# nipponjo/tts-arabic-pytorch

Hardware: AMD Instinct MI355X
Metric: audio samples/sec (FastPitch+HiFi-GAN, synthetic 64-phoneme inputs) (higher is better)
Workload: dtype f32

## Files before the change

### include/ttsamd.h

```cpp
#ifndef TTSAMD_H
#define TTSAMD_H

#include <stdint.h>

#ifdef __cplusplus
extern "C" {
#endif

#define TTSAMD_OK 0
#define TTSAMD_EINVAL (-1)
#define TTSAMD_EHIP (-2)
#define TTSAMD_ENOMEM (-3)

typedef struct ttsamd_tensor {
    const char* name;
    const float* data;
    int32_t ndim;
    int64_t shape[4];
} ttsamd_tensor;

typedef struct ttsamd_hifigan_cfg {
    int32_t num_mels;
    int32_t upsample_initial_channel;
    int32_t n_ups;
// ... 260 lines not shown

int64_t ttsamd_conv1d_packed_floats(int32_t cout, int32_t cin, int32_t k);
int32_t ttsamd_conv1d(const float* x, const float* w, const float* bias, const int64_t* lens,
                      int32_t batch, int32_t cin, int32_t cout, int32_t k, int32_t dilation,
                      int32_t lin, float in_slope, int32_t relu_out, float* y, float* packed,
                      void* stream);
int32_t ttsamd_conv1d_ex(const float* x, const float* w, const float* bias, const float* res, const int64_t* lens, int32_t batch,
                         int32_t cin, int32_t cout, int32_t k, int32_t dilation, int32_t lin, float in_slope,
                         int32_t relu_out, int32_t mode, float div, float* y, float* packed, void* stream);
int32_t ttsamd_conv1d_splitk(const float* x, const float* w, const float* bias, const float* res, const int64_t* lens, int32_t batch,
                             int32_t cin, int32_t cout, int32_t k, int32_t dilation, int32_t lin, float in_slope,
                             int32_t relu_out, int32_t mode, float div, float* y, float* packed, float* splitk_ws, int64_t splitk_floats,
                             void* stream);
int32_t ttsamd_conv_last_launch(int32_t* route, int32_t* ksplit);
int64_t ttsamd_convt_packed_floats(int32_t cin, int32_t cout, int32_t u);
int32_t ttsamd_conv_transpose1d(const float* x, const float* w, const float* bias, const int64_t* lens, int32_t batch, int32_t cin,
                                int32_t cout, int32_t u, int32_t lin, float in_slope, float* y, float* packed, void* stream);

int64_t ttsamd_resblock_pair_packed_floats(int32_t channels, int32_t k, int32_t variant);
int32_t ttsamd_resblock_pair(const float* x, float* y, const float* w1, const float* b1, const float* w2, const float* b2,
                             int32_t channels, int32_t k, int32_t dil, const int64_t* lens, int32_t len_mul, int32_t L,
                             int32_t batch, int32_t mode, float div, float slope, int32_t variant, float* packed, int64_t packed_floats,
                             void* stream);

int64_t ttsamd_resblock2_packed_floats(int32_t channels, int32_t k, int32_t variant);
int32_t ttsamd_resblock2(const float* x, float* y, const float* w1, const float* b1, const float* w2, const float* b2, int32_t channels,
                         int32_t k, int32_t dil1, int32_t dil2, const int64_t* lens, int32_t len_mul, int32_t L, int32_t batch, int32_t mode,
                         float div, float slope, int32_t variant, float* packed, int64_t packed_floats, void* stream);

int32_t ttsamd_bfo_pack(const float* x, int32_t batch, int32_t channels, int32_t len, float slope, void* out, void* stream);
// ... 97 lines not shown
```

### tts-arabic-pytorch_amd/csrc/api.hip

```cpp
#include <cerrno>
#include <cstdio>
#include <cstdlib>
#include <cstring>
#include <algorithm>
#include <atomic>
#include <mutex>
#include <string>
#include <vector>

#include "kernels.hpp"

namespace ttsamd {

static thread_local std::string g_err;

void set_error(const char* fmt, ...) {
    char buf[1024];
    va_list ap;
    va_start(ap, fmt);
    vsnprintf(buf, sizeof(buf), fmt, ap);
    va_end(ap);
    g_err = buf;
}

// ... 158 lines not shown

__global__ void pack_convt_weight_kernel(const float* __restrict__ w, int cin, int cout, int u, int cp, float* __restrict__ out) {
    const int64_t i = (int64_t)blockIdx.x * 256 + threadIdx.x;
    const int64_t n = (int64_t)u * cin * 2 * cp;
    if (i >= n) return;
    const int pq = (int)(i % 4);
    const int co = (int)((i / 4) % cp);
    const int kk = (int)((i / (4 * (int64_t)cp)) % 2);
    const int t = (int)((i / (8 * (int64_t)cp)) % 2);
    const int o = (int)((i / (16 * (int64_t)cp)) % (cin / 8));
    const int rho = (int)(i / (16 * (int64_t)cp * (cin / 8)));
    const int kidx = (rho + u / 2) % u + t * u;
    out[i] = co < cout ? w[((int64_t)(8 * o + 2 * pq + kk) * cout + co) * (2 * u) + kidx] : 0.f;
}

__global__ void split_bf16_kernel(const float* __restrict__ packed, int64_t n, unsigned short* __restrict__ out) {
    const int64_t i = (int64_t)blockIdx.x * 256 + threadIdx.x;
    if (i >= n) return;
    const float f = packed[i];
    unsigned u = __float_as_uint(f);
    u += 0x7fffu + ((u >> 16) & 1u);
    const unsigned h = u >> 16;
    const float r = f - __uint_as_float(h << 16);
    unsigned v = __float_as_uint(r);
    v += 0x7fffu + ((v >> 16) & 1u);
    out[i] = (unsigned short)h;
    out[n + i] = (unsigned short)(v >> 16);
}

namespace {
// ... 645 lines not shown

int32_t ttsamd_conv1d(const float* x, const float* w, const float* bias, const int64_t* lens, int32_t batch,
                      int32_t cin, int32_t cout, int32_t k, int32_t dilation, int32_t lin, float in_slope,
                      int32_t relu_out, float* y, float* packed, void* stream) {
    return ttsamd_conv1d_ex(x, w, bias, nullptr, lens, batch, cin, cout, k, dilation, lin, in_slope, relu_out, 0, 1.f, y, packed, stream);
}

int32_t ttsamd_conv_last_launch(int32_t* route, int32_t* ksplit) {
    TTS_REQUIRE(route && ksplit, "conv_last_launch: null argument");
    last_conv_launch(route, ksplit);
    return 0;
}

int64_t ttsamd_convt_packed_floats(int32_t cin, int32_t cout, int32_t u) {
    if (cin < 1 || cout < 1 || u < 1) return 0;
    return 2 * (int64_t)u * cin * 2 * cout_padded(cout);
}

int32_t ttsamd_conv_transpose1d(const float* x, const float* w, const float* bias, const int64_t* lens, int32_t batch, int32_t cin,
                                int32_t cout, int32_t u, int32_t lin, float in_slope, float* y, float* packed, void* stream) {
    TTS_REQUIRE(x && w && y && packed, "conv_transpose1d: null argument");
    TTS_REQUIRE(batch >= 1 && cin >= 8 && cin % 8 == 0 && cout >= 1 && lin >= 1, "conv_transpose1d: batch %d, cin %d (a multiple of 8), cout %d, lin %d",
                batch, cin, cout, lin);
    TTS_REQUIRE(u >= 2 && u % 2 == 0, "conv_transpose1d: stride %d (kernel 2 u, padding u / 2: u even)", u);
    TTS_REQUIRE((int64_t)lin * u < ((int64_t)1 << 31) / 4 / cout, "conv_transpose1d: %d x %d x %d outputs per row", cout, lin, u);
    hipStream_t s = (hipStream_t)stream;
    const int cp = cout_padded(cout);
    const int64_t n = (int64_t)u * cin * 2 * cp;
    hipLaunchKernelGGL(pack_convt_weight_kernel, dim3((unsigned)((n + 255) / 256)), dim3(256), 0, s, w, cin, cout, u, cp, packed);
    TTS_CHECK_HIP(hipGetLastError());
    unsigned short* planes = nullptr;
    if (default_precision() != 0) {
        planes = reinterpret_cast<unsigned short*>(packed + n);
        hipLaunchKernelGGL(split_bf16_kernel, dim3((unsigned)((n + 255) / 256)), dim3(256), 0, s, packed, n, planes);
        TTS_CHECK_HIP(hipGetLastError());
    }
    ConvParams p;
    std::memset(&p, 0, sizeof(p));
    p.batch = batch;
    p.lens_in = lens; p.lens_out = lens;
    prof_begin(s, 2.0 * cout * cin * 2 * u);
    const int32_t rc = launch_upsampler(p, x, packed, planes, bias, y, cin, cout, u, 2 * u, lin, 1, in_slope, opt_int(OPT_CONVT, 1) != 0, s);
    prof_end(s);
    return rc;
}

int64_t ttsamd_resblock_pair_packed_floats(int32_t channels, int32_t k, int32_t variant) {
    if (channels < 1 || k < 1) return 0;
    const int64_t n = 2 * (int64_t)channels * k * channels;
    const int nwino = (variant == 4 ? 1 : (variant == 5 ? 2 : 0));
    if (variant == 6) return n + ((k == 3 || k == 7 || k == 11) ? 2 * (int64_t)channels * wino4_groups(k) * channels : 0);
    return n + ((k == 3 || k == 7 || k == 11) ? nwino * (int64_t)channels * wino2_groups(k) * channels : 0);
}

int32_t ttsamd_resblock_pair(const float* x, float* y, const float* w1, const float* b1, const float* w2, const float* b2,
                             int32_t channels, int32_t k, int32_t dil, const int64_t* lens, int32_t len_mul, int32_t L,
                             int32_t batch, int32_t mode, float div, float slope, int32_t variant, float* packed, int64_t packed_floats,
// ... 151 lines not shown
```

### tts-arabic-pytorch_amd/csrc/common.hpp

```cpp
#pragma once
#include <hip/hip_runtime.h>
#include <stdint.h>
#include <atomic>
#include <cstdarg>
#include <cstdio>
#include <cstdlib>
#include <string>

#include "../../include/ttsamd.h"

namespace ttsamd {

void set_error(const char* fmt, ...);

#define TTS_CHECK_HIP(expr)                                                         \
    do {                                                                            \
        hipError_t e_ = (expr);                                                     \
        if (e_ != hipSuccess) {                                                     \
            ttsamd::set_error("%s failed: %s (%s:%d)", #expr, hipGetErrorString(e_), \
                              __FILE__, __LINE__);                                  \
            return TTSAMD_EHIP;                                                     \
        }                                                                           \
    } while (0)

// ... 23 lines not shown
    return e;
}

#define TTS_OPTIONS(X)                                                                                     \
    X(HIFIGAN_STREAMS, 0, 0, 1)    \
    X(WINO, 0, 0, 1)                                              \
    X(WINO2, 0, 0, 31)             \
    X(WINO4, 0, 0, 127)            \
    X(FUSED_PAIR, 0, 0, 1)                   \
    X(FUSED2, 0, 0, 1)                                           \
    X(FUSED2_MASK, 1, 0, 0x1ff)               \
    X(FUSED2_MASK_N1, 1, 0, 0x1ff)          \
    X(FUSED2_WB, 0, 0, 2)                     \
    X(PAIR4, 0, 0, 1)              \
    X(CONVT, 0, 0, 1)                              \
    X(BFO, 0, 0, 1)                \
    X(BFO_CHAIN, 0, 0, 1)                           \
    X(BFO_CHAIN7, 0, 0, 1)                                 \
    X(BFO_FF, 0, 0, 1)                              \
    X(BFO_SPLITK, 0, 0, 1)                                              \
    X(BFO_SMALL_TILES, 0, 0, 1)            \
    X(BF16_ATTN, 0, 0, 1)                                         \
    X(BF16_PACKED_T, 0, 0, 1)                   \
    X(ATT_RA, 0, 1, 4)                             \
    X(ATT_SPLIT, 0, 0, 1)                      \
    X(XCD_W, 0, 0, 1)                            \
    X(XCD_WMAX_KB, 0, 0, 1 << 20)     \
    X(DEEP_SPLITK, 0, 0, 1)        \
    X(TACO_PERSISTENT, 0, 0, 2)    \
    X(TACO_SEG, 0, 8, 1 << 20)     \
// ... 64 lines not shown
    unsigned long long* timing;
    const float* w_wino44;
};
constexpr int64_t kSplitKFloats = 4 << 20;
constexpr int64_t kSplitKFloatsFp = 8 << 20;

void conv_log(const char* kind, int K, int cin, int cout, int nout, int batch, int has_res, int mode, int len_mul, int ragged,
              int n_phase);
bool compact_order(const void* lens, int batch);
int32_t launch_conv(const ConvParams& p, hipStream_t stream);
void note_conv_launch(int32_t route, int32_t ksplit);
void last_conv_launch(int32_t* route, int32_t* ksplit);
bool convt_supported(const ConvParams& p);
int32_t launch_convt(const ConvParams& p, hipStream_t stream);
int32_t launch_upsampler(ConvParams& p, const float* x, const float* w, const void* w_bf16, const float* bias, float* y, int cin, int cout,
                         int u, int kt, int L, int len_mul, float in_slope, bool convt_ok, hipStream_t stream);
bool fused_pair_supported(int32_t channels, int32_t k, int32_t dil, int32_t L, const float* x, const float* y);
int32_t launch_fused_pair(int32_t channels, const float* x, float* y, const float* w1, const float* b1, const float* w2,
                          const float* b2, int32_t k, int32_t dil, const int64_t* lens, int32_t len_mul, int32_t L, int32_t batch,
                          int32_t mode, float div, float slope, hipStream_t stream);
bool fused_pair2_supported(int32_t channels, int32_t k, int32_t dil, int32_t L, const float* x, const float* y, int32_t ntw);
int32_t launch_fused_pair2(int32_t channels, const float* x, float* y, const float* w1, const float* b1, const float* w2,
                           const float* b2, int32_t k, int32_t dil, const int64_t* lens, int32_t len_mul, int32_t L, int32_t batch,
                           int32_t mode, float div, float slope, int32_t ntw, hipStream_t stream, const float* w2_wino = nullptr,
                           const float* w1_wino = nullptr);
bool fused_pair4_supported(int32_t channels, int32_t k, int32_t dil, int32_t L, const float* x, const float* y);
int32_t launch_fused_pair4(int32_t channels, const float* x, float* y, const float* w1_wino4, const float* b1, const float* w2_wino4,
                           const float* b2, int32_t k, int32_t dil, const int64_t* lens, int32_t len_mul, int32_t L, int32_t batch,
                           int32_t mode, float div, float slope, hipStream_t stream);
bool resblock2_conv_supported(int32_t channels, int32_t k, int32_t dil, int32_t L, const float* x, const float* y);
int32_t launch_resblock2_conv(int32_t channels, const float* x, float* y, const float* w, const float* b, int32_t k, int32_t dil,
// ... 17 lines not shown
int wino4_block_outputs(int dil);
int wino4_ksplit(const ConvParams& p);
int32_t launch_splitk_reduce(const ConvParams& q, hipStream_t stream);
int32_t launch_wino4(const ConvParams& p, hipStream_t stream);
void wino4_filter_groups(const float* g, int k, float* o);
void pack_wino4_weight(const float* w, int cout, int cin, int k, float* out);
void wino44_filter_groups(const float* g, int k, float* o);
void pack_wino44_weight(const float* w, int cout, int cin, int k, float* out);
void pack_conv_weight(const float* w, int cout, int cin, int k, float* out);
void pack_convt_weight(const float* w, int cin, int cout, int kt, int u, int p, float* out);
inline int cout_padded(int cout) { return (int)align_up(cout, 32); }
void split_packed_bf16(const float* packed, int64_t n, uint16_t* out);
int32_t default_precision();

#ifdef __HIPCC__
__device__ __forceinline__ bool live_tile(const int64_t* __restrict__ lens, const int mul, const int n_max, const int tile_w,
                                          const int batch, const unsigned lin, int& b, int& tile) {
    const int lane = threadIdx.x & 63;
    unsigned base = 0;
    for (int u0 = 0; u0 < batch; u0 += 64) {
        int n = 0;
        if (u0 + lane < batch) n = (max(min(n_max, (int)lens[u0 + lane] * mul), 0) + tile_w - 1) / tile_w;
        int incl = n;
#pragma unroll
        for (int d = 1; d < 64; d <<= 1) {
            const int t = __shfl_up(incl, d, 64);
            if (lane >= d) incl += t;
        }
        const unsigned total = (unsigned)__shfl(incl, 63, 64);
        if (lin < base + total) {
            const unsigned long long m = __ballot(base + (unsigned)incl > lin);
            const int l = __ffsll((long long)m) - 1;
            b = u0 + l;
            tile = (int)(lin - base) - (__shfl(incl, l, 64) - __shfl(n, l, 64));
            return true;
        }
        base += total;
// ... 7 lines not shown
```

### tts-arabic-pytorch_amd/csrc/conv_wino4.hip

```cpp
#include <cstdlib>
#include <cstring>

#include <algorithm>
#include <vector>

#include "conv_mfma_common.hpp"
#include "bfo.hpp"

namespace ttsamd {

typedef float w4_f32x4 __attribute__((ext_vector_type(4)));
typedef float w4_f32x2 __attribute__((ext_vector_type(2)));

template <int K, int NOCT_, int NSTAGE_, int PT_ = 6, int LP_ = 1>
struct Wino4Geo {
    static constexpr bool PT7 = PT_ == 7;
    static_assert(PT_ == 6 || (PT7 && (K == 7 || K == 11)), "seven-point groups: k = 7 / 11");
    static constexpr int WM = 2, WN = 2;
    static constexpr int NSF = K == 1 ? 0 : (K == 3 ? 1 : (K == 7 ? 2 : (PT7 ? 3 : 4)));
    static constexpr int NL = (!PT7 && (K == 7 || K == 1)) ? 1 : 0;
    static constexpr int GSF = PT7 ? 7 : 6;
    static constexpr int SSF = PT7 ? 4 : 3;
    static constexpr int NG = PT7 ? (K == 7 ? 13 : 20) : (K == 1 ? 4 : (K == 3 ? 6 : (K == 7 ? 16 : 23)));
    static constexpr int NGQ = PT7 ? NG : ((NG + 1) & ~1);
    static constexpr bool WSHARE = K == 1;
    static constexpr int NGW = WSHARE ? 1 : NGQ;
    static constexpr int NPL = PT7 ? 7 : (NL ? 8 : 6);
    static constexpr int NPOS = K == 1 ? 4 : (K == 3 ? 6 : (K == 7 ? 10 : 14));
    static constexpr int NOCT = NOCT_, NSTAGE = NSTAGE_;
    static constexpr int NPH = PT7 ? ((K == 11 && LP_ == 2) ? 2 : 1) : (K == 11 ? 2 : 1);
    static constexpr int PH0 = PT7 ? 8 : 12;
    static constexpr int NGPM = NPH == 1 ? NG : 12;
    static_assert(NPH == 1 || (PH0 <= NGPM && NG - PH0 <= NGPM), "phase sizes");
    static constexpr int CO_BLK = WM * 32;
    static constexpr int NTUP = WN * 32;
    static constexpr int NT_BLK = 4 * NTUP;
    static constexpr int BUF4 = NOCT * 2 * NGPM * NTUP;
    static constexpr int PF = 4;
    static constexpr int NM = 4;
    __host__ __device__ static constexpr int glo(int ph) { return NPH == 1 ? 0 : PH0 * ph; }
    __host__ __device__ static constexpr int ngp(int ph) { return NPH == 1 ? NG : (ph == 0 ? PH0 : NG - PH0); }
    __host__ __device__ static constexpr int ngq(int ph) { return NPH == 1 ? NGQ : (PT7 ? ngp(ph) : 12); }
    __host__ __device__ static constexpr int gfirst(int g) {
// ... 49 lines not shown
    __host__ __device__ static constexpr int wst(int ph) { return (sgap(ph) - tw0t(ph)) / nwj(ph); }
    static_assert(LP_ != 2 || (wst(0) >= 1 && wst(NPH - 1) >= 1), "one write job per gap at most (strip path)");
    static constexpr int QX = WSHARE ? 0 : (NOCT * ngq(0)) % PF;
    static constexpr int QMAIN = NOCT * ngq(0) - QX;
    static_assert(QX == 0 || (NPH == 1 && NOCT == 1 && QMAIN >= 2 * PF), "extra queue slots: one phase, one octet");
    static_assert((WSHARE ? NOCT : NOCT * ngq(NPH - 1)) % PF == 0 || QX != 0, "queue slots line up across steps");
    static_assert((size_t)NSTAGE * BUF4 * 16 + (LP_ == 2 ? RAW_BYTES : 0) <= 80 * 1024, "two blocks per CU");
    static_assert(NPH == 1 || NOCT == 1, "phases split an octet's groups");
};

__device__ __host__ constexpr int wino4_tile(int d, int ntup) { return (4 * ntup / (4 * d)) * (4 * d); }

template <int K, int NOCT_, int NSTAGE_, int EPI, int LP, int PT = 6>
__global__ __launch_bounds__(256, kConvMinWaves) void conv1d_wino4_f32(const ConvParams p) {
    extern __shared__ __attribute__((aligned(16))) float4 smem4[];
    using G = Wino4Geo<K, NOCT_, NSTAGE_, PT, LP>;
    constexpr bool PT7 = G::PT7;
    constexpr int WN = G::WN, NSF = G::NSF, NOCT = G::NOCT, NSTAGE = G::NSTAGE, NPL = G::NPL, NGPM = G::NGPM;
    constexpr int CO_BLK = G::CO_BLK, NTUP = G::NTUP, NT_BLK = G::NT_BLK, PF = G::PF;
    constexpr int NPH = G::NPH, NPOSP = G::NPOSP, NM = G::NM;
    constexpr bool D1 = LP == 1, TR = LP == 2;
    static_assert(D1 || TR, "window path");
    const int dil = D1 ? 1 : p.dil;
    const int nt_eff = wino4_tile(dil, NTUP), ntup_eff = nt_eff / 4;
    const int tiles_y = p.CoutP / CO_BLK;
    const int per_tile = tiles_y * p.ksplit;
    const unsigned sidx = blockIdx.x, xcd = sidx & 7u, u = sidx >> 3;
    const int yk = (int)(u % (unsigned)per_tile);
    const unsigned gt = (u / (unsigned)per_tile) * 8u + xcd;
    const int n_tiles_x = (p.Nout + nt_eff - 1) / nt_eff;
    int b = (int)(gt / (unsigned)n_tiles_x);
    int q0 = (int)(gt % (unsigned)n_tiles_x) * nt_eff;
    if (p.compact) {
        int tile = 0;
        if (!live_tile(p.lens_out, p.len_out_mul, p.Nout, nt_eff, p.batch, gt, b, tile)) return;
        b = __builtin_amdgcn_readfirstlane(b);
        q0 = __builtin_amdgcn_readfirstlane(tile) * nt_eff;
    } else if (b >= p.batch) {
        return;
    }
    const int tid = threadIdx.x, lane = tid & 63, wid = tid >> 6;
    const int wm = wid / WN, wn = wid % WN;
    const int ks = yk / tiles_y;
    const int co_blk0 = (yk - ks * tiles_y) * CO_BLK;
    int n_out = p.Nout;
    if (p.lens_out) n_out = min(n_out, (int)p.lens_out[b] * p.len_out_mul);
    if (q0 >= n_out) return;
    int in_len = p.Lin;
    if (p.lens_in) in_len = min(in_len, (int)p.lens_in[b] * p.len_in_mul);

    const int x_cs = p.x_cs, CoutP = p.CoutP;
    const int chunks_all = p.Cin / (8 * NOCT);
    const int c_beg = (int)((int64_t)ks * chunks_all / p.ksplit), n_chunks = (int)((int64_t)(ks + 1) * chunks_all / p.ksplit);
    const int n_groups = (p.Cin / 8) * G::NGW;
    const float* __restrict__ xb = p.x + (int64_t)b * p.x_bs;
    const float in_slope = p.in_slope;

    constexpr bool REG = EPI >= 3, RES = EPI == 3;
    static_assert(!REG || (LP == 1 && K != 1), "register epilogue: dilation 1, k = 3 / 7 / 11");
    float ep_bias = 0.f;
    if constexpr (!REG) {
        if (tid < CO_BLK && p.bias) ep_bias = p.bias[min(co_blk0 + tid, p.Cout - 1)];
    }

    const int kk = lane >> 5, l31 = lane & 31;
    const int pe = wn * 32 + l31;
    const int col_e = dil == 1 ? 4 * pe : (pe / dil) * 4 * dil + pe % dil;
    f32x16 acc[NPL];
#pragma unroll
    for (int g = 0; g < NPL; ++g)
#pragma unroll
        for (int r = 0; r < 16; ++r) acc[g][r] = 0.f;
    const int ep_row0 = REG ? co_blk0 + __builtin_amdgcn_readfirstlane(wm) * 32 : 0;
    const int ep_voff = (q0 + col_e < n_out ? q0 + col_e : 0) * 4;
// ... 279 lines not shown
        float y0 = acc[0][R] + s12 + s34;                                                            \
        float y1 = d12 + 2.f * d34;                                                                  \
        float y2 = s12 + 4.f * s34;                                                                  \
        float y3 = d12 + 8.f * d34 + acc[PT7 ? 6 : 5][R];                                            \
        if constexpr (NSF == 0) { y0 = acc[0][R]; y1 = 0.f; y2 = 0.f; y3 = acc[5][R]; }               \
        if constexpr (PT7) {                                                                   \
            y0 += acc[5][R];                                                                         \
            y1 += 0.5f * acc[5][R];                                                                  \
            y2 += 0.25f * acc[5][R];                                                                 \
            y3 += 0.125f * acc[5][R];                                                                \
        } else if constexpr (NPL == 8) {                                                             \
            y1 += acc[6][R];                                                                         \
            y2 += acc[7][R];                                                                         \
        }
    float* __restrict__ yb = p.y + (int64_t)b * p.y_bs;
    const int mode = p.mode, relu_out = p.relu_out, Cout = p.Cout;
    const float div = p.div;
    if constexpr (REG) {
        const int q = q0 + col_e, y_cs = p.y_cs;
        if (q >= n_out) return;
        const bool full = q + 3 < n_out;
        const bfo_i4 ys = bfo_rsrc(yb, (unsigned)Cout * (unsigned)y_cs * 4u);
        const float lo = relu_out == 1 ? 0.f : -__builtin_inff();
        constexpr int PB = NPL >= 8 ? 4 : 8;
#pragma unroll
        for (int h = 0; h < 16 / PB; ++h) {
            w4_f32x4 pq[PB];
#pragma unroll
            for (int i = 0; i < PB; ++i) {
                const int r = PB * h + i;
// ... 205 lines not shown
    return ((int)opt_int(OPT_WINO4, kWino4Default) & (p.K == 7 ? 32 : 64)) != 0;
}

int32_t launch_wino4(const ConvParams& p, hipStream_t stream) {
    if (wino44_wanted(p)) return p.K == 7 ? launch_wino44_cfg<7>(p, stream) : launch_wino44_cfg<11>(p, stream);
    if (p.K == 1) return launch_wino4_epi<1, 4, 2, 0, 1>(p, stream);
    if (p.K == 3) return launch_wino4_cfg<3, 2, 3>(p, stream);
    if (p.K == 7) return launch_wino4_cfg<7, 1, 2>(p, stream);
    if (p.K == 11) return launch_wino4_cfg<11, 1, 3>(p, stream);
    set_error("wino4: kernel size %d not built (1, 3, 7, 11)", p.K);
    return TTSAMD_EINVAL;
}

int wino4_block_outputs(int dil) { return wino4_tile(dil, 64); }

int wino4_ksplit(const ConvParams& p) {
    const int bo = wino4_block_outputs(p.dil);
    const int64_t blocks = (int64_t)((p.Nout + bo - 1) / bo) * (p.CoutP / 64) * p.batch;
    constexpr int sk_blocks = 192, sk_target = 224;
    if (blocks >= sk_blocks || p.splitk_ws == nullptr) return 1;
    const int n_chunks = p.Cin / (p.K == 1 ? 32 : (p.K == 3 ? 16 : 8));
    const int64_t per = (int64_t)p.batch * p.Cout * p.Nout;
    int64_t ks = std::min<int64_t>((sk_target + blocks - 1) / blocks, n_chunks / 8);
    ks = std::min<int64_t>(ks, p.splitk_floats / std::max<int64_t>(per, 1));
    return ks >= 2 ? (int)ks : 1;
}

int wino4_groups(int k) { return k == 3 ? 6 : (k == 7 ? 16 : 24); }
int wino44_groups(int k) { return k == 7 ? 13 : (k == 11 ? 20 : 0); }

// ... 45 lines not shown
```

### tts-arabic-pytorch_amd/csrc/convt_mfma.hip

```cpp
#include <cstring>

#include <cstdlib>
#include "conv_mfma_common.hpp"

namespace ttsamd {

template <int U, int MT, int NTL, int WM>
struct ConvtGeo {
    static constexpr int WN = 4 / WM;
    static constexpr int CO_BLK = WM * MT * 32;
    static constexpr int NT_BLK = WN * NTL * 32;
    static constexpr int XS = NT_BLK + 2;
    static constexpr int X4 = 2 * XS;
    static constexpr int W4 = U * 4 * CO_BLK;
    static constexpr int STG4 = X4 + W4;
    static constexpr int NW = (W4 + 255) / 256;
    static constexpr int NX = (X4 + 255) / 256;
};

template <int U, int MT, int NTL, int WM>
__global__ __launch_bounds__(256, 2) void convt_mfma_f32(const ConvParams p) {
    using G = ConvtGeo<U, MT, NTL, WM>;
    constexpr int WN = G::WN, CO_BLK = G::CO_BLK, NT_BLK = G::NT_BLK, XS = G::XS, NW = G::NW, NX = G::NX;
    extern __shared__ __attribute__((aligned(16))) float4 smem4[];
// ... 173 lines not shown
           p.scale == nullptr && p.relu_out == 0 && p.Cin % 8 == 0 && !p.x_packed && !p.y_packed &&
           (p.y_cs % 4) == 0 && (p.y_bs % 4) == 0 && (((uintptr_t)p.y) & 15) == 0 &&
           (p.n_phase == 8 ? p.CoutP % 64 == 0 : p.CoutP % 32 == 0);
}

int32_t launch_convt(const ConvParams& p, hipStream_t stream) {
    TTS_REQUIRE(convt_supported(p), "convt: unsupported geometry");
    if (p.Nout <= 0) return 0;
    conv_log("convt", 2, p.Cin, p.Cout, p.Nout, p.batch, 0, 0, p.len_out_mul, p.lens_out != nullptr, p.n_phase);
    note_conv_launch(5, 1);
    if (p.n_phase == 8) return launch_convt_cfg<8, 1, 1, 2>(p, stream);
    if (p.CoutP % 64 == 0) return launch_convt_cfg<2, 1, 2, 2>(p, stream);
    return launch_convt_cfg<2, 1, 4, 1>(p, stream);
}

int32_t launch_upsampler(ConvParams& p, const float* x, const float* w, const void* w_bf16, const float* bias, float* y, int cin, int cout,
                         int u, int kt, int L, int len_mul, float in_slope, bool convt_ok, hipStream_t stream) {
    p.x = x; p.x_bs = (int64_t)cin * L; p.x_cs = L;
    p.w = w; p.bias = bias;
    p.w_bf16 = w_bf16; p.precision = default_precision(); p.w_wino = nullptr; p.w_wino4 = nullptr; p.w_wino44 = nullptr;
    p.y = y; p.y_bs = (int64_t)cout * L * u; p.y_cs = L * u; p.y_ts = u;
    p.res = nullptr;
    p.len_in_mul = len_mul; p.len_out_mul = len_mul; p.Lin = L; p.Nout = L;
    p.Cin = cin; p.Cout = cout; p.CoutP = cout_padded(cout); p.K = 2;
    p.dil = -1; p.pad = 0; p.n_phase = u; p.phase_p = (kt - u) / 2;
    p.in_slope = in_slope; p.relu_out = 0; p.mode = 0; p.div = 1.f;
    p.x_packed = 0; p.y_packed = 0;
    return (convt_ok && convt_supported(p)) ? launch_convt(p, stream) : launch_conv(p, stream);
}

}
```

### tts-arabic-pytorch_amd/csrc/hifigan.hip

```cpp
#include <cmath>
#include <cstring>
#include <cstdlib>
#include <map>
#include <mutex>
#include <string>
#include <vector>

#include "kernels.hpp"
#include "bfo.hpp"

namespace ttsamd {

constexpr unsigned kFused2Mask = 0x00F;
constexpr int kPair4MinK = 7;
constexpr unsigned kFused2MaskN1 = 0x000;
constexpr int64_t kFused2SmallColumns = 2 * 256 * 252;

constexpr unsigned kResblock2PairMask = 0x00;

static bool resblock2_pair_choice(unsigned mask, int32_t channels, int32_t k, int32_t d1, int32_t d2, int32_t L, const float* x,
                                  const float* y) {
    const int ci = channels == 32 ? 0 : (channels == 64 ? 1 : -1);
    const int ki = k == 3 ? 0 : (k == 5 ? 1 : (k == 7 ? 2 : -1));
    if (ci < 0 || ki < 0 || !(mask & (1u << (3 * ci + ki)))) return false;
    return resblock2_pair_supported(channels, k, d1, d2, L, x, y);
}

struct ConvW {
    int64_t w_off = 0, b_off = 0;
    int64_t w16_off = 0, w_n = 0;
    BfoWeightOffs wo;
    int64_t ww44_off = -1;
    int64_t ww4_off = -1;
    int64_t ww_off = -1;
    int cin = 0, cout = 0, k = 0;
};

struct HifiGan {
    ttsamd_hifigan_cfg cfg;
    float* dev = nullptr;
    uint16_t* dev16 = nullptr;
    int64_t dev_n = 0, dev16_n = 0;
    ConvW conv_pre, conv_post;
    std::vector<ConvW> ups;
    std::vector<ConvW> c1, c2;
    int hop = 1;
    bool rb2 = false;
    int64_t max_cl = 0;
// ... 194 lines not shown
            set_error("hifigan: ups.%d has shape [%lld,%lld,%lld], expected [%d,%d,%d]", i, (long long)shp[0],
                      (long long)shp[1], (long long)shp[2], cin, cout, kt);
            rc = TTSAMD_EINVAL;
            break;
        }
        ConvW cw;
        cw.cin = cin; cw.cout = cout; cw.k = kt;
        cw.w_off = (int64_t)blob.size();
        blob.resize(blob.size() + (size_t)u * cin * 2 * cout_padded(cout));
        pack_convt_weight(w.data(), cin, cout, kt, u, (kt - u) / 2, blob.data() + cw.w_off);
        add_bf16(blob, blob16, cw, (int64_t)u * cin * 2 * cout_padded(cout));
        if (cin % 16 == 0 && cout % 32 == 0 && (u == 8 || u == 2)) cw.wo = bfo_append_weights(w.data(), cout, cin, kt, u, blob16);
        blob.resize(align_up((int64_t)blob.size(), 64));
        rc = get_bias(tm, "ups." + std::to_string(i), cout, blob, cw.b_off);
        if (rc) break;
        h->ups.push_back(cw);
        ch = cout;
        mul *= u;
        h->max_cl = std::max<int64_t>(h->max_cl, (int64_t)ch * mul);
        for (int j = 0; rc == 0 && j < cfg->n_kernels; ++j) {
            const int r = i * cfg->n_kernels + j, kk = cfg->resblock_kernel_sizes[j];
            if (h->rb2) {
                if (!resblock2_conv_supported(ch, kk, cfg->resblock_dilations[j][0], 1, nullptr, blob.data()) ||
                    !resblock2_conv_supported(ch, kk, cfg->resblock_dilations[j][1], 1, nullptr, blob.data())) {
                    set_error("hifigan: ResBlock2 at C = %d, k = %d, dilations %d / %d is not built (C = 32 / 64 / 128, k = 3 / 5 / 7 / 11, "
                              "dilation 1..16)", ch, kk, cfg->resblock_dilations[j][0], cfg->resblock_dilations[j][1]);
                    rc = TTSAMD_EINVAL;
                    break;
                }
                ConvW a, b;
// ... 292 lines not shown
                in_section = false;
                prof_section_end(s);
            }
        }
        HG_TRY(M.conv_post(curo, h->dev + h->conv_post.w_off, h->dev + h->conv_post.b_off, lens, mul, B, h->conv_post.cin, L, wave, (int64_t)L, s));
        return 0;
    }

    HG_TRY(conv(h->conv_pre, mel, s, cur, nullptr, T, 1, 1, 1.0f, 0, 1.f));
    int L = T, mul = 1;
    for (int i = 0; i < cfg.n_ups; ++i) {
        const int u = cfg.upsample_rates[i], kt = cfg.upsample_kernel_sizes[i];
        const ConvW& uw = h->ups[i];
        prof_begin(s, 2.0 * uw.cout * uw.cin * 2 * u * mul);
        int32_t rc = launch_upsampler(p, cur, h->dev + uw.w_off, h->dev16 + uw.w16_off, h->dev + uw.b_off, ups_out, uw.cin, uw.cout, u, kt, L,
                                      mul, 0.1f, convt_ok, s);
        prof_end(s);
        HG_TRY(rc);
        L *= u; mul *= u;
        if (multi) {
            prof_section_begin(s);
            in_section = true;
            HG_CHECK_HIP(hipEventRecord(h->ev_fork, s));
        }
        for (int j = 0; h->rb2 && j < cfg.n_kernels; ++j) {
            hipStream_t st = bs[j % 3];
            float* Tb = Tbs[j % 3];
            if (multi && j > 0) HG_CHECK_HIP(hipStreamWaitEvent(st, h->ev_fork, 0));
            const int r = i * cfg.n_kernels + j;
            const ConvW &w1 = h->c1[r], &w2 = h->c2[r];
            const int d1 = cfg.resblock_dilations[j][0], d2 = cfg.resblock_dilations[j][1];
// ... 105 lines not shown
```

### tts-arabic-pytorch_amd/ttsamd/lib.py

```python
import ctypes as C
import os

_HERE = os.path.dirname(os.path.abspath(__file__))
LIB_PATH = os.environ.get('TTSAMD_LIB') or os.path.join(_HERE, 'lib', 'libttsamd.so')


class TtsAmdError(RuntimeError):
    pass


class Tensor(C.Structure):
    _fields_ = [('name', C.c_char_p), ('data', C.POINTER(C.c_float)), ('ndim', C.c_int32),
                ('shape', C.c_int64 * 4)]


class HifiGanCfg(C.Structure):
    _fields_ = [('num_mels', C.c_int32), ('upsample_initial_channel', C.c_int32), ('n_ups', C.c_int32),
                ('upsample_rates', C.c_int32 * 8), ('upsample_kernel_sizes', C.c_int32 * 8),
                ('n_kernels', C.c_int32), ('resblock_kernel_sizes', C.c_int32 * 8),
                ('n_dilations', C.c_int32), ('resblock_dilations', (C.c_int32 * 8) * 8), ('resblock', C.c_int32)]


class FastPitchCfg(C.Structure):
    _fields_ = [(n, C.c_int32) for n in (
# ... 126 lines not shown
    'ttsamd_tacotron2_destroy': (_I32, [_P]),
    'ttsamd_tacotron2_workspace_bytes': (_I64, [_P, _I32, _I32, _I32]),
    'ttsamd_tacotron2_infer': (_I32, [_P, _P, _P, _P, _I32, _I32, _I32, _I64, _P, _P, _P, _P,
                                      C.POINTER(_I32), _P, _I64, _P]),
    'ttsamd_tagger_create': (_I32, [C.POINTER(Tensor), _I32, C.POINTER(TaggerCfg), C.POINTER(_P)]),
    'ttsamd_tagger_destroy': (_I32, [_P]),
    'ttsamd_tagger_workspace_bytes': (_I64, [_P, _I32, _I32]),
    'ttsamd_tagger_forward': (_I32, [_P, _P, _I32, _I32, _P, _P, _I64, _P]),
    'ttsamd_conv1d_packed_floats': (_I64, [_I32, _I32, _I32]),
    'ttsamd_conv1d': (_I32, [_P, _P, _P, _P, _I32, _I32, _I32, _I32, _I32, _I32, _F, _I32, _P, _P, _P]),
    'ttsamd_conv1d_ex': (_I32, [_P, _P, _P, _P, _P, _I32, _I32, _I32, _I32, _I32, _I32, _F, _I32, _I32, _F, _P, _P, _P]),
    'ttsamd_conv1d_splitk': (_I32, [_P, _P, _P, _P, _P, _I32, _I32, _I32, _I32, _I32, _I32, _F, _I32, _I32, _F, _P, _P, _P, _I64, _P]),
    'ttsamd_conv_last_launch': (_I32, [C.POINTER(_I32), C.POINTER(_I32)]),
    'ttsamd_convt_packed_floats': (_I64, [_I32, _I32, _I32]),
    'ttsamd_conv_transpose1d': (_I32, [_P, _P, _P, _P, _I32, _I32, _I32, _I32, _I32, _F, _P, _P, _P]),
    'ttsamd_resblock_pair_packed_floats': (_I64, [_I32, _I32, _I32]),
    'ttsamd_resblock_pair': (_I32, [_P, _P, _P, _P, _P, _P, _I32, _I32, _I32, _P, _I32, _I32, _I32, _I32, _F, _F, _I32, _P, _I64, _P]),
    'ttsamd_resblock2_packed_floats': (_I64, [_I32, _I32, _I32]),
    'ttsamd_resblock2': (_I32, [_P, _P, _P, _P, _P, _P, _I32, _I32, _I32, _I32, _P, _I32, _I32, _I32, _I32, _F, _F, _I32, _P, _I64, _P]),
    'ttsamd_set_precision': (_I32, [_I32]),
    'ttsamd_get_precision': (_I32, []),
    'ttsamd_dp_unique_id': (_I32, [_P]),
    'ttsamd_dp_init': (_I32, [_I32, _I32, _P, C.POINTER(_P)]),
    'ttsamd_dp_destroy': (_I32, [_P]),
    'ttsamd_dp_rank': (_I32, [_P]),
    'ttsamd_dp_world': (_I32, [_P]),
    'ttsamd_dp_broadcast': (_I32, [_P, _P, _I64, _I32, _P]),
    'ttsamd_dp_broadcast_weights': (_I32, [_P, _I32, _P, _I32, _P]),
    'ttsamd_dp_allgather': (_I32, [_P, _P, _P, _I64, _P]),
    'ttsamd_dp_pack_audio': (_I32, [_P, _I64, _P, _I32, _I64, _P, _P]),
# ... 111 lines not shown
```

Baseline: 77.01 million.

## Route HiFi-GAN transposed-conv upsamplers through Winograd F(4,3) kernel

Recasts the stride-u transposed convolution (kernel 2u, padding u/2) as a k=3 dilation-1 convolution with u*cout output rows, using five Winograd points instead of six. It reuses the existing wino4 conv kernel with new transposed-conv epilogues that scatter outputs into the upsampled layout. The transformed weights and biases are packed once at model load. This is meant to cut the multiply count of the upsampler layers. It adds new epilogue store paths with boundary handling, a positions threshold that decides when the path is taken, and extra weight memory.

```diff
diff --git a/include/ttsamd.h b/include/ttsamd.h
--- a/include/ttsamd.h
+++ b/include/ttsamd.h
@@ -298,6 +298,8 @@
                              void* stream);
 int32_t ttsamd_conv_last_launch(int32_t* route, int32_t* ksplit);
 int64_t ttsamd_convt_packed_floats(int32_t cin, int32_t cout, int32_t u);
+int64_t ttsamd_convt_wino_packed_floats(int32_t cin, int32_t cout, int32_t u);
+int32_t ttsamd_convt_wino_pack_weight(const float* w, const float* bias, int32_t cin, int32_t cout, int32_t u, float* out);
 int32_t ttsamd_conv_transpose1d(const float* x, const float* w, const float* bias, const int64_t* lens, int32_t batch, int32_t cin,
                                 int32_t cout, int32_t u, int32_t lin, float in_slope, float* y, float* packed, void* stream);
 
diff --git a/tts-arabic-pytorch_amd/csrc/api.hip b/tts-arabic-pytorch_amd/csrc/api.hip
--- a/tts-arabic-pytorch_amd/csrc/api.hip
+++ b/tts-arabic-pytorch_amd/csrc/api.hip
@@ -196,6 +196,30 @@
     out[i] = co < cout ? w[((int64_t)(8 * o + 2 * pq + kk) * cout + co) * (2 * u) + kidx] : 0.f;
 }
 
+__global__ void pack_convt_wino_kernel(const float* __restrict__ w, const float* __restrict__ bias, int cin, int cout, int u,
+                                       float* __restrict__ out) {
+    const int64_t i = (int64_t)blockIdx.x * 256 + threadIdx.x;
+    const int rows = u * cout;
+    const int64_t n = (int64_t)6 * cin * rows;
+    if (i >= n + rows) return;
+    if (i >= n) {
+        out[i] = bias ? bias[(i - n) / u] : 0.f;
+        return;
+    }
+    const int pq = (int)(i & 3);
+    const int64_t r = i >> 2;
+    const int row = (int)(r % rows);
+    const int64_t r2 = r / rows;
+    const int kk = (int)(r2 & 1);
+    const int64_t r3 = r2 >> 1;
+    const int t = (int)(r3 % 6), o = (int)(r3 / 6);
+    const int co = row / u, j = row % u;
+    const float* g = w + ((int64_t)(8 * o + 2 * pq + kk) * cout + co) * 2 * u;
+    const double g0 = g[j + u], g1 = g[j];
+    out[i] = t == 0 ? (float)(g0 / 4) : (t == 1 ? (float)(-(g0 + g1) / 6) : (t == 2 ? (float)(-(g0 - g1) / 6) :
+             (t == 3 ? (float)(g0 / 24 + g1 / 12) : (t == 4 ? (float)(g0 / 24 - g1 / 12) : 0.f))));
+}
+
 __global__ void split_bf16_kernel(const float* __restrict__ packed, int64_t n, unsigned short* __restrict__ out) {
     const int64_t i = (int64_t)blockIdx.x * 256 + threadIdx.x;
     if (i >= n) return;
@@ -871,7 +895,19 @@
 
 int64_t ttsamd_convt_packed_floats(int32_t cin, int32_t cout, int32_t u) {
     if (cin < 1 || cout < 1 || u < 1) return 0;
-    return 2 * (int64_t)u * cin * 2 * cout_padded(cout);
+    return 2 * (int64_t)u * cin * 2 * cout_padded(cout) + (convt_wino_packable(cin, cout, u) ? (int64_t)(6 * cin + 1) * u * cout : 0);
+}
+
+int64_t ttsamd_convt_wino_packed_floats(int32_t cin, int32_t cout, int32_t u) {
+    return convt_wino_packable(cin, cout, u) ? (int64_t)(6 * cin + 1) * u * cout : 0;
+}
+
+int32_t ttsamd_convt_wino_pack_weight(const float* w, const float* bias, int32_t cin, int32_t cout, int32_t u, float* out) {
+    TTS_REQUIRE(w && out, "convt_wino_pack_weight: null argument");
+    TTS_REQUIRE(convt_wino_packable(cin, cout, u), "convt_wino_pack_weight: cin %d (a multiple of 16), cout %d, u %d (2 / 8, u cout a multiple of 64)",
+                cin, cout, u);
+    pack_convt_wino_weight(w, bias, cin, cout, u, out, out + (int64_t)6 * cin * u * cout);
+    return 0;
 }
 
 int32_t ttsamd_conv_transpose1d(const float* x, const float* w, const float* bias, const int64_t* lens, int32_t batch, int32_t cin,
@@ -892,12 +928,20 @@
         hipLaunchKernelGGL(split_bf16_kernel, dim3((unsigned)((n + 255) / 256)), dim3(256), 0, s, packed, n, planes);
         TTS_CHECK_HIP(hipGetLastError());
     }
+    float* wino = nullptr;
+    if (default_precision() == 0 && convt_wino_packable(cin, cout, u) && opt_int(OPT_CONVT_WINO, 1) != 0) {
+        wino = packed + 2 * n;
+        const int64_t nw = (int64_t)(6 * cin + 1) * u * cout;
+        hipLaunchKernelGGL(pack_convt_wino_kernel, dim3((unsigned)((nw + 255) / 256)), dim3(256), 0, s, w, bias, cin, cout, u, wino);
+        TTS_CHECK_HIP(hipGetLastError());
+    }
     ConvParams p;
     std::memset(&p, 0, sizeof(p));
     p.batch = batch;
     p.lens_in = lens; p.lens_out = lens;
     prof_begin(s, 2.0 * cout * cin * 2 * u);
-    const int32_t rc = launch_upsampler(p, x, packed, planes, bias, y, cin, cout, u, 2 * u, lin, 1, in_slope, opt_int(OPT_CONVT, 1) != 0, s);
+    const int32_t rc = launch_upsampler(p, x, packed, planes, bias, y, cin, cout, u, 2 * u, lin, 1, in_slope, opt_int(OPT_CONVT, 1) != 0, s, wino,
+                                        wino ? wino + (int64_t)6 * cin * u * cout : nullptr);
     prof_end(s);
     return rc;
 }
diff --git a/tts-arabic-pytorch_amd/csrc/common.hpp b/tts-arabic-pytorch_amd/csrc/common.hpp
--- a/tts-arabic-pytorch_amd/csrc/common.hpp
+++ b/tts-arabic-pytorch_amd/csrc/common.hpp
@@ -61,6 +61,7 @@
     X(FUSED2_WB, 0, 0, 2)                     \
     X(PAIR4, 0, 0, 1)              \
     X(CONVT, 0, 0, 1)                              \
+    X(CONVT_WINO, 0, 0, 2)         \
     X(BFO, 0, 0, 1)                \
     X(BFO_CHAIN, 0, 0, 1)                           \
     X(BFO_CHAIN7, 0, 0, 1)                                 \
@@ -155,7 +156,12 @@
 bool convt_supported(const ConvParams& p);
 int32_t launch_convt(const ConvParams& p, hipStream_t stream);
 int32_t launch_upsampler(ConvParams& p, const float* x, const float* w, const void* w_bf16, const float* bias, float* y, int cin, int cout,
-                         int u, int kt, int L, int len_mul, float in_slope, bool convt_ok, hipStream_t stream);
+                         int u, int kt, int L, int len_mul, float in_slope, bool convt_ok, hipStream_t stream, const float* w_wino = nullptr,
+                         const float* bias_wino = nullptr);
+bool convt_wino_packable(int cin, int cout, int u);
+void pack_convt_wino_weight(const float* w, const float* bias, int cin, int cout, int u, float* out_w, float* out_bias);
+bool convt_wino_supported(const ConvParams& p, const float* w_wino, const float* bias_wino);
+int32_t launch_convt_wino(const ConvParams& p, const float* w_wino, const float* bias_wino, hipStream_t stream);
 bool fused_pair_supported(int32_t channels, int32_t k, int32_t dil, int32_t L, const float* x, const float* y);
 int32_t launch_fused_pair(int32_t channels, const float* x, float* y, const float* w1, const float* b1, const float* w2,
                           const float* b2, int32_t k, int32_t dil, const int64_t* lens, int32_t len_mul, int32_t L, int32_t batch,
@@ -203,13 +209,21 @@
 int32_t default_precision();
 
 #ifdef __HIPCC__
+template <int EXTRA = 0>
 __device__ __forceinline__ bool live_tile(const int64_t* __restrict__ lens, const int mul, const int n_max, const int tile_w,
                                           const int batch, const unsigned lin, int& b, int& tile) {
     const int lane = threadIdx.x & 63;
     unsigned base = 0;
     for (int u0 = 0; u0 < batch; u0 += 64) {
         int n = 0;
-        if (u0 + lane < batch) n = (max(min(n_max, (int)lens[u0 + lane] * mul), 0) + tile_w - 1) / tile_w;
+        if constexpr (EXTRA != 0) {
+            if (u0 + lane < batch) {
+                const int len = (int)lens[u0 + lane] * mul;
+                n = (max(min(n_max, len > 0 ? len + EXTRA : 0), 0) + tile_w - 1) / tile_w;
+            }
+        } else {
+            if (u0 + lane < batch) n = (max(min(n_max, (int)lens[u0 + lane] * mul), 0) + tile_w - 1) / tile_w;
+        }
         int incl = n;
 #pragma unroll
         for (int d = 1; d < 64; d <<= 1) {
diff --git a/tts-arabic-pytorch_amd/csrc/conv_wino4.hip b/tts-arabic-pytorch_amd/csrc/conv_wino4.hip
--- a/tts-arabic-pytorch_amd/csrc/conv_wino4.hip
+++ b/tts-arabic-pytorch_amd/csrc/conv_wino4.hip
@@ -12,21 +12,22 @@
 typedef float w4_f32x4 __attribute__((ext_vector_type(4)));
 typedef float w4_f32x2 __attribute__((ext_vector_type(2)));
 
-template <int K, int NOCT_, int NSTAGE_, int PT_ = 6, int LP_ = 1>
+template <int K, int NOCT_, int NSTAGE_, int PT_ = 6, int LP_ = 1, int CT_ = 0>
 struct Wino4Geo {
     static constexpr bool PT7 = PT_ == 7;
     static_assert(PT_ == 6 || (PT7 && (K == 7 || K == 11)), "seven-point groups: k = 7 / 11");
+    static_assert(CT_ == 0 || (K == 3 && PT_ == 6 && LP_ == 1), "transposed conv: the k = 3 six-point form at dilation 1");
     static constexpr int WM = 2, WN = 2;
     static constexpr int NSF = K == 1 ? 0 : (K == 3 ? 1 : (K == 7 ? 2 : (PT7 ? 3 : 4)));
     static constexpr int NL = (!PT7 && (K == 7 || K == 1)) ? 1 : 0;
     static constexpr int GSF = PT7 ? 7 : 6;
     static constexpr int SSF = PT7 ? 4 : 3;
-    static constexpr int NG = PT7 ? (K == 7 ? 13 : 20) : (K == 1 ? 4 : (K == 3 ? 6 : (K == 7 ? 16 : 23)));
+    static constexpr int NG = PT7 ? (K == 7 ? 13 : 20) : (K == 1 ? 4 : (K == 3 ? (CT_ ? 5 : 6) : (K == 7 ? 16 : 23)));
     static constexpr int NGQ = PT7 ? NG : ((NG + 1) & ~1);
     static constexpr bool WSHARE = K == 1;
     static constexpr int NGW = WSHARE ? 1 : NGQ;
-    static constexpr int NPL = PT7 ? 7 : (NL ? 8 : 6);
-    static constexpr int NPOS = K == 1 ? 4 : (K == 3 ? 6 : (K == 7 ? 10 : 14));
+    static constexpr int NPL = PT7 ? 7 : (NL ? 8 : (CT_ ? 5 : 6));
+    static constexpr int NPOS = K == 1 ? 4 : (K == 3 ? (CT_ ? 5 : 6) : (K == 7 ? 10 : 14));
     static constexpr int NOCT = NOCT_, NSTAGE = NSTAGE_;
     static constexpr int NPH = PT7 ? ((K == 11 && LP_ == 2) ? 2 : 1) : (K == 11 ? 2 : 1);
     static constexpr int PH0 = PT7 ? 8 : 12;
@@ -106,7 +107,9 @@
 template <int K, int NOCT_, int NSTAGE_, int EPI, int LP, int PT = 6>
 __global__ __launch_bounds__(256, kConvMinWaves) void conv1d_wino4_f32(const ConvParams p) {
     extern __shared__ __attribute__((aligned(16))) float4 smem4[];
-    using G = Wino4Geo<K, NOCT_, NSTAGE_, PT, LP>;
+    constexpr int CTU = EPI == 5 ? 8 : (EPI == 6 ? 2 : 0);
+    constexpr bool CT = CTU != 0;
+    using G = Wino4Geo<K, NOCT_, NSTAGE_, PT, LP, CTU>;
     constexpr bool PT7 = G::PT7;
     constexpr int WN = G::WN, NSF = G::NSF, NOCT = G::NOCT, NSTAGE = G::NSTAGE, NPL = G::NPL, NGPM = G::NGPM;
     constexpr int CO_BLK = G::CO_BLK, NTUP = G::NTUP, NT_BLK = G::NT_BLK, PF = G::PF;
@@ -125,7 +128,7 @@
     int q0 = (int)(gt % (unsigned)n_tiles_x) * nt_eff;
     if (p.compact) {
         int tile = 0;
-        if (!live_tile(p.lens_out, p.len_out_mul, p.Nout, nt_eff, p.batch, gt, b, tile)) return;
+        if (!live_tile<CT ? 1 : 0>(p.lens_out, p.len_out_mul, p.Nout, nt_eff, p.batch, gt, b, tile)) return;
         b = __builtin_amdgcn_readfirstlane(b);
         q0 = __builtin_amdgcn_readfirstlane(tile) * nt_eff;
     } else if (b >= p.batch) {
@@ -136,7 +139,14 @@
     const int ks = yk / tiles_y;
     const int co_blk0 = (yk - ks * tiles_y) * CO_BLK;
     int n_out = p.Nout;
-    if (p.lens_out) n_out = min(n_out, (int)p.lens_out[b] * p.len_out_mul);
+    if constexpr (CT) {
+        if (p.lens_out) {
+            const int len = min(p.Lin, (int)p.lens_out[b] * p.len_out_mul);
+            n_out = len > 0 ? len + 1 : 0;
+        }
+    } else {
+        if (p.lens_out) n_out = min(n_out, (int)p.lens_out[b] * p.len_out_mul);
+    }
     if (q0 >= n_out) return;
     int in_len = p.Lin;
     if (p.lens_in) in_len = min(in_len, (int)p.lens_in[b] * p.len_in_mul);
@@ -150,6 +160,7 @@
 
     constexpr bool REG = EPI >= 3, RES = EPI == 3;
     static_assert(!REG || (LP == 1 && K != 1), "register epilogue: dilation 1, k = 3 / 7 / 11");
+    static_assert(EPI <= 6 && (!CT || K == 3), "epilogues 0, 3, 4 and the transposed conv's 5 / 6 (k = 3 form)");
     float ep_bias = 0.f;
     if constexpr (!REG) {
         if (tid < CO_BLK && p.bias) ep_bias = p.bias[min(co_blk0 + tid, p.Cout - 1)];
@@ -459,6 +470,67 @@
             y2 += acc[7][R];                                                                         \
         }
     float* __restrict__ yb = p.y + (int64_t)b * p.y_bs;
+    if constexpr (CT) {
+        const int tau0 = q0 + col_e, y_cs = p.y_cs;
+        if constexpr (CTU == 8) {
+            if (tau0 >= n_out) return;
+        }
+        const int olen = CTU * (n_out - 1);
+        const int ch0 = ep_row0 / CTU;
+#define TTS_CT_QUAD(R, Y)                                                                            \
+        {                                                                                            \
+            const float s12 = acc[1][R] + acc[2][R], d12 = acc[1][R] - acc[2][R];                    \
+            const float s34 = acc[3][R] + acc[4][R], d34 = acc[3][R] - acc[4][R];                    \
+            (Y)[0] = acc[0][R] + s12 + s34;                                                          \
+            (Y)[1] = d12 + 2.f * d34;                                                                \
+            (Y)[2] = s12 + 4.f * s34;                                                                \
+            (Y)[3] = d12 + 8.f * d34;                                                                \
+        }
+        if constexpr (CTU == 8) {
+#pragma unroll
+            for (int c = 0; c < 4; ++c) {
+                float yq[4][4];
+#pragma unroll
+                for (int i = 0; i < 4; ++i) TTS_CT_QUAD(4 * c + i, yq[i])
+                float* yr = yb + (int64_t)(ch0 + c) * y_cs;
+#pragma unroll
+                for (int e = 0; e < 4; ++e) {
+                    const int n = 8 * (tau0 + e) + 4 * kk - 4;
+                    if (n >= 0 && n < olen)
+                        *reinterpret_cast<w4_f32x4*>(yr + n) = w4_f32x4{yq[0][e] + bsq[c][0], yq[1][e] + bsq[c][1], yq[2][e] + bsq[c][2], yq[3][e] + bsq[c][3]};
+                }
+            }
+        } else {
+#pragma unroll
+            for (int m = 0; m < 8; ++m) {
+                float ya[4], yc[4];
+                TTS_CT_QUAD(2 * m, ya)
+                TTS_CT_QUAD(2 * m + 1, yc)
+                const float b0 = bsq[m >> 1][(2 * m) & 3], b1 = bsq[m >> 1][(2 * m + 1) & 3];
+                const float v[8] = {ya[0] + b0, yc[0] + b1, ya[1] + b0, yc[1] + b1, ya[2] + b0, yc[2] + b1, ya[3] + b0, yc[3] + b1};
+                const int n0 = 2 * tau0 - 1;
+                float* yr = yb + (int64_t)(ch0 + 2 * kk + (m & 1) + 4 * (m >> 1)) * y_cs + n0;
+                const float nb = __shfl_down(v[0], 1, 64);
+                const bool has_nb = l31 != 31;
+                if (l31 == 0 && n0 >= 0 && n0 < olen) yr[0] = v[0];
+                if (n0 + 8 < olen) {
+                    *reinterpret_cast<w4_f32x4*>(yr + 1) = w4_f32x4{v[1], v[2], v[3], v[4]};
+                    if (has_nb) {
+                        *reinterpret_cast<w4_f32x4*>(yr + 5) = w4_f32x4{v[5], v[6], v[7], nb};
+                    } else {
+                        *reinterpret_cast<w4_f32x2*>(yr + 5) = w4_f32x2{v[5], v[6]};
+                        yr[7] = v[7];
+                    }
+                } else {
+#pragma unroll
+                    for (int e = 1; e < 8; ++e)
+                        if (n0 + e < olen) yr[e] = v[e];
+                }
+            }
+        }
+#undef TTS_CT_QUAD
+        return;
+    }
     const int mode = p.mode, relu_out = p.relu_out, Cout = p.Cout;
     const float div = p.div;
     if constexpr (REG) {
@@ -694,6 +766,63 @@
 
 int wino4_block_outputs(int dil) { return wino4_tile(dil, 64); }
 
+bool convt_wino_packable(int cin, int cout, int u) { return (u == 2 || u == 8) && cin >= 16 && cin % 16 == 0 && cout >= 1 && (u * cout) % 64 == 0; }
+
+bool convt_wino_supported(const ConvParams& p, const float* w_wino, const float* bias_wino) {
+    const int u = p.n_phase;
+    return w_wino != nullptr && bias_wino != nullptr && p.precision == 0 && convt_wino_packable(p.Cin, p.Cout, u) && p.K == 2 && p.dil == -1 &&
+           p.phase_p * 2 == u && p.y_ts == u && p.res == nullptr && p.mode == 0 && p.scale == nullptr && p.relu_out == 0 &&
+           !p.x_packed && !p.y_packed && p.in_slope >= 0.f && p.in_slope <= 1.f && p.Lin == p.Nout &&
+           (p.x_cs & 3) == 0 && (p.x_bs & 3) == 0 && ((uintptr_t)p.x & 15) == 0 &&
+           (p.y_cs & 3) == 0 && (p.y_bs & 3) == 0 && ((uintptr_t)p.y & 15) == 0 &&
+           (int64_t)p.Lin * 4 + 64 < ((int64_t)1 << 31) && (int64_t)p.Cout * p.y_cs * 4 < ((int64_t)1 << 31);
+}
+
+template <int U>
+static int32_t launch_convt_wino_u(const ConvParams& p, const float* w_wino, const float* bias_wino, hipStream_t stream) {
+    constexpr int EPI = U == 8 ? 5 : 6;
+    using G = Wino4Geo<3, 2, 3, 6, 1, U>;
+    constexpr size_t lds = (size_t)G::NSTAGE * G::BUF4 * sizeof(float4);
+    static_assert(lds <= 80 * 1024, "two blocks per CU");
+    static std::atomic<uint64_t> lds_done{0};
+    const auto kern = conv1d_wino4_f32<3, 2, 3, EPI, 1, 6>;
+    TTS_CHECK_HIP(lds_opt_in((const void*)kern, (int)lds, lds_done));
+    ConvParams q = p;
+    q.w_wino4 = w_wino; q.bias = bias_wino;
+    q.Cout = U * p.Cout; q.CoutP = q.Cout;
+    q.Nout = p.Lin + 1;
+    q.K = 3; q.dil = 1; q.pad = 1; q.n_phase = 1; q.ksplit = 1;
+    const int64_t n_tiles = (int64_t)((q.Nout + G::NT_BLK - 1) / G::NT_BLK) * p.batch;
+    const int64_t n_blocks = ((n_tiles + 7) / 8) * 8 * (q.CoutP / G::CO_BLK);
+    TTS_REQUIRE(n_blocks < ((int64_t)1 << 31), "convt wino: %lld blocks", (long long)n_blocks);
+    q.compact = compact_order(p.lens_out, p.batch) ? 1 : 0;
+    hipLaunchKernelGGL(kern, dim3((unsigned)n_blocks, 1, 1), dim3(256), lds, stream, q);
+    TTS_CHECK_HIP(hipGetLastError());
+    return 0;
+}
+
+int32_t launch_convt_wino(const ConvParams& p, const float* w_wino, const float* bias_wino, hipStream_t stream) {
+    TTS_REQUIRE(convt_wino_supported(p, w_wino, bias_wino), "convt wino: unsupported geometry");
+    if (p.Nout <= 0) return 0;
+    conv_log("convt_wino", 2, p.Cin, p.Cout, p.Nout, p.batch, 0, 0, p.len_out_mul, p.lens_out != nullptr, p.n_phase);
+    note_conv_launch(6, 1);
+    return p.n_phase == 8 ? launch_convt_wino_u<8>(p, w_wino, bias_wino, stream) : launch_convt_wino_u<2>(p, w_wino, bias_wino, stream);
+}
+
+void pack_convt_wino_weight(const float* w, const float* bias, int cin, int cout, int u, float* out_w, float* out_bias) {
+    const int rows = u * cout;
+    std::vector<float> t((size_t)rows * cin * 3);
+    for (int ci = 0; ci < cin; ++ci)
+        for (int co = 0; co < cout; ++co)
+            for (int j = 0; j < u; ++j) {
+                const float* g = w + ((int64_t)ci * cout + co) * 2 * u;
+                float* d = t.data() + ((int64_t)(co * u + j) * cin + ci) * 3;
+                d[0] = g[j + u]; d[1] = g[j]; d[2] = 0.f;
+            }
+    pack_wino4_weight(t.data(), rows, cin, 3, out_w);
+    for (int r = 0; r < rows; ++r) out_bias[r] = bias ? bias[r / u] : 0.f;
+}
+
 int wino4_ksplit(const ConvParams& p) {
     const int bo = wino4_block_outputs(p.dil);
     const int64_t blocks = (int64_t)((p.Nout + bo - 1) / bo) * (p.CoutP / 64) * p.batch;
diff --git a/tts-arabic-pytorch_amd/csrc/convt_mfma.hip b/tts-arabic-pytorch_amd/csrc/convt_mfma.hip
--- a/tts-arabic-pytorch_amd/csrc/convt_mfma.hip
+++ b/tts-arabic-pytorch_amd/csrc/convt_mfma.hip
@@ -211,8 +211,15 @@
     return launch_convt_cfg<2, 1, 4, 1>(p, stream);
 }
 
+constexpr int64_t kConvtWinoMinPositions = 8192;
+static bool convt_wino_default(int cin, int u, int64_t positions) {
+    if (positions < kConvtWinoMinPositions) return false;
+    return (u == 8 && (cin == 512 || cin == 256)) || (u == 2 && (cin == 128 || cin == 64));
+}
+
 int32_t launch_upsampler(ConvParams& p, const float* x, const float* w, const void* w_bf16, const float* bias, float* y, int cin, int cout,
-                         int u, int kt, int L, int len_mul, float in_slope, bool convt_ok, hipStream_t stream) {
+                         int u, int kt, int L, int len_mul, float in_slope, bool convt_ok, hipStream_t stream, const float* w_wino,
+                         const float* bias_wino) {
     p.x = x; p.x_bs = (int64_t)cin * L; p.x_cs = L;
     p.w = w; p.bias = bias;
     p.w_bf16 = w_bf16; p.precision = default_precision(); p.w_wino = nullptr; p.w_wino4 = nullptr; p.w_wino44 = nullptr;
@@ -223,6 +230,10 @@
     p.dil = -1; p.pad = 0; p.n_phase = u; p.phase_p = (kt - u) / 2;
     p.in_slope = in_slope; p.relu_out = 0; p.mode = 0; p.div = 1.f;
     p.x_packed = 0; p.y_packed = 0;
+    const int64_t wino = opt_int(OPT_CONVT_WINO, 1);
+    if (convt_ok && wino != 0 && kt == 2 * u && convt_wino_supported(p, w_wino, bias_wino) &&
+        (wino == 2 || convt_wino_default(cin, u, (int64_t)p.batch * L)))
+        return launch_convt_wino(p, w_wino, bias_wino, stream);
     return (convt_ok && convt_supported(p)) ? launch_convt(p, stream) : launch_conv(p, stream);
 }
 
diff --git a/tts-arabic-pytorch_amd/csrc/hifigan.hip b/tts-arabic-pytorch_amd/csrc/hifigan.hip
--- a/tts-arabic-pytorch_amd/csrc/hifigan.hip
+++ b/tts-arabic-pytorch_amd/csrc/hifigan.hip
@@ -32,6 +32,7 @@
     BfoWeightOffs wo;
     int64_t ww44_off = -1;
     int64_t ww4_off = -1;
+    int64_t wct_off = -1, bct_off = -1;
     int64_t ww_off = -1;
     int cin = 0, cout = 0, k = 0;
 };
@@ -256,6 +257,13 @@
         blob.resize(align_up((int64_t)blob.size(), 64));
         rc = get_bias(tm, "ups." + std::to_string(i), cout, blob, cw.b_off);
         if (rc) break;
+        if (convt_wino_packable(cin, cout, u)) {
+            cw.wct_off = (int64_t)blob.size();
+            blob.resize(blob.size() + (size_t)6 * cin * u * cout);
+            cw.bct_off = (int64_t)blob.size();
+            blob.resize(align_up((int64_t)blob.size() + (int64_t)u * cout, 64));
+            pack_convt_wino_weight(w.data(), blob.data() + cw.b_off, cin, cout, u, blob.data() + cw.wct_off, blob.data() + cw.bct_off);
+        }
         h->ups.push_back(cw);
         ch = cout;
         mul *= u;
@@ -578,7 +586,8 @@
         const ConvW& uw = h->ups[i];
         prof_begin(s, 2.0 * uw.cout * uw.cin * 2 * u * mul);
         int32_t rc = launch_upsampler(p, cur, h->dev + uw.w_off, h->dev16 + uw.w16_off, h->dev + uw.b_off, ups_out, uw.cin, uw.cout, u, kt, L,
-                                      mul, 0.1f, convt_ok, s);
+                                      mul, 0.1f, convt_ok, s, uw.wct_off >= 0 ? h->dev + uw.wct_off : nullptr,
+                                      uw.bct_off >= 0 ? h->dev + uw.bct_off : nullptr);
         prof_end(s);
         HG_TRY(rc);
         L *= u; mul *= u;
diff --git a/tts-arabic-pytorch_amd/ttsamd/lib.py b/tts-arabic-pytorch_amd/ttsamd/lib.py
--- a/tts-arabic-pytorch_amd/ttsamd/lib.py
+++ b/tts-arabic-pytorch_amd/ttsamd/lib.py
@@ -164,6 +164,8 @@
     'ttsamd_conv_last_launch': (_I32, [C.POINTER(_I32), C.POINTER(_I32)]),
     'ttsamd_convt_packed_floats': (_I64, [_I32, _I32, _I32]),
     'ttsamd_conv_transpose1d': (_I32, [_P, _P, _P, _P, _I32, _I32, _I32, _I32, _I32, _F, _P, _P, _P]),
+    'ttsamd_convt_wino_packed_floats': (_I64, [_I32, _I32, _I32]),
+    'ttsamd_convt_wino_pack_weight': (_I32, [_P, _P, _I32, _I32, _I32, _P]),
     'ttsamd_resblock_pair_packed_floats': (_I64, [_I32, _I32, _I32]),
     'ttsamd_resblock_pair': (_I32, [_P, _P, _P, _P, _P, _P, _I32, _I32, _I32, _P, _I32, _I32, _I32, _I32, _F, _F, _I32, _P, _I64, _P]),
     'ttsamd_resblock2_packed_floats': (_I64, [_I32, _I32, _I32]),
```

After: 78.39 million (median of 6 runs). +1.8%, better.
